# 91Mrwu/sif-xco2-cokriging

Hardware: AMD Instinct MI355X
Metric: cokriging grid-points/s at n_obs=20k bivariate (higher is better)
Workload: dtype f64; 1 GPU; configs[2]: n_obs=20000/process (N=40000) SIF+XCO2-like residuals on the 0.05-degree CONUS lattice, haversine, full 2n x 2n solve, 8833-point 0.5-degree grid, Matern set A; n_obs=20000, N=40000, m=8833, partition=block-column-cyclic x1

## Files before the change

sif-xco2-cokriging_amd/csrc/ck_api.hip:

```cpp
#include <hip/hip_runtime.h>
#include <math.h>
#include <stdio.h>
#include <string.h>

#include <algorithm>
#include <cmath>
#include <atomic>
#include <memory>
#include <string>
#include <utility>
#include <thread>
#include <vector>

#include "../../include/cokrige.h"
#include "ck_devbuf.h"
#include "ck_host.h"
#include "ck_internal.h"
#include "ck_tilemap.h"
#include "ck_model.h"
#include "ck_vecchia.h"

static int64_t roundup(int64_t x, int64_t a) { return (x + a - 1) / a * a; }
#define CK_N_TIMINGS 118
#define CK_TREND_TOL 1e-10
// ... 111 lines not shown
    int64_t p_cap = 0;
    DevBuf<char[24]> mv_buf;
    AuxState aux_state = AUX_NONE;
    double par_sigma[2] = {0.0, 0.0}, par_rho = 0.0;
    DevBuf<CkMatern> d_lik_blk;
    CkMatern lik_hb[15];
    DevBuf<double> baux;
    int64_t block_chunk = 0;
    int64_t sim_free_bytes = 0;
    int64_t draw_chunk = 0;
    struct Schur {
        int64_t M = 0;
        int tiles = 0;
        std::vector<DevBuf<double>> panels;
        std::vector<double*> sig;
        DevBuf<double*> d_ptr, d_coefptr;
        DevBuf<int> d_tile0, d_panel_of;
        DevBuf<double> pc, c, u;
        DevBuf<CkMatern> d_blk;
        DevBuf<CkTable> d_tabs;
        DevBuf<long long> d_info;
    } sch;
    std::vector<double> vg_ci, vg_cj, vg_vi, vg_vj;
    struct Vario {
        DevBuf<double> iu, iv, ju_own, jv_own;
        double *ju = nullptr, *jv = nullptr;
        DevBuf<unsigned long long> best;
        DevBuf<double> jb, ib64, jbsub;
        DevBuf<CkVarioExt> part;
        DevBuf<double> psum;
        DevBuf<unsigned long long> pcnt;
        DevBuf<double> out;
        DevBuf<CkVarioPair> list;
        DevBuf<unsigned> count;
    } vg;
    int64_t vg_ni = 0, vg_nj = 0;
    int vg_same = 0, vg_bgrid = 0;
    int64_t vg_stats[4] = {0, 0, 0, 0};
    double t_ms[CK_N_TIMINGS] = {};
    int time_gemm = 0;
    std::vector<EvPair> gemm_ev;
    size_t gemm_ev_used = 0;
    hipEvent_t ev0 = nullptr, ev1 = nullptr, ev2 = nullptr, ev3 = nullptr;
    hipStream_t side = nullptr;
    hipStream_t side_lo = nullptr;
    int fused_sweeps_opt = -1;
    int fused_prio = 0;
    int fused_group = 0;
    int group_first = -1, group_tail = 0, group_tail_panels = 0;
    int assemble_queue = -1;
    int tall_sweep = 1;
    int tall_split = 2;
    int tall_split_rows = 24 * CK_NB;
    int solve_la = -1;
    int tall_b2_stream = 1;
    std::vector<hipEvent_t> ev_b2;
    int tall_thin = 1;
    int fused_la = -1;
    std::vector<hipEvent_t> ev_col, ev_pan;
    int panel_group = 0;
    int64_t local_slab_mb = 0;
    int local_tile_min = 64;
    int64_t local_nmax[2] = {0, 0};
    int local_select_cap = 0;
    int local_group = 4;
    int local_left = 1;
    int panel_fused = 2 | 16;
    int64_t loo_g0 = -1;
    DevBuf<double> d_chunkb;
    DevBuf<double> local_slab;
    int lookahead = -1;
    DevBuf<unsigned> d_coop;
    DevBuf<unsigned long long> d_stamps;
    size_t n_stamps = 0;
    int64_t stamp_grid[4] = {0, 0, 0, 0};
    int stamp_sel = 0;
    unsigned coop_seq = 0;
    unsigned coop_spins = 2000000;
    int coop_inject_panel = -1;
    std::vector<double> trend_F[2];
    int trend_p[2] = {0, 0};
    bool trend_dirty = false;
    DevBuf<double> d_trendX;
    DevBuf<double> d_univ;
    std::vector<double> noise_var[2];
    double noise_scale[2] = {1.0, 1.0};
    bool noise_dirty = false, noise_on = false;
    DevBuf<double> d_noise;
    double lik_noise_grad[2] = {0.0, 0.0};
    bool lik_noise_valid = false;
    int aux_trend = 0;
    int loo_dense = 1;
    int64_t fisher_product_mb = 0;

    ~ck_handle() {
        for (auto& e : gemm_ev) {
            (void)hipEventDestroy(e.a);
            (void)hipEventDestroy(e.b);
        }
        for (hipEvent_t e : {ev0, ev1, ev2, ev3})
            if (e) (void)hipEventDestroy(e);
        for (const auto* v : {&ev_b2, &ev_col, &ev_pan})
            for (hipEvent_t e : *v) (void)hipEventDestroy(e);
        for (hipStream_t st : {side, side_lo, own_stream})
            if (st) (void)hipStreamDestroy(st);
    }
// ... 682 lines not shown
}
static void gemm_timed_end(ck_handle* h, hipStream_t st = nullptr) {
    if (!st) st = h->stream;
    if (!h->time_gemm) return;
    (void)hipEventRecord(h->gemm_ev[h->gemm_ev_used].b, st);
    h->gemm_ev_used++;
}

static void gemm_timed_collect(ck_handle* h, int slot, hipEvent_t ref = nullptr) {
    if (!h->time_gemm) return;
    double tot = 0;
    std::vector<std::pair<float, float>> iv;
    for (size_t e = 0; e < h->gemm_ev_used; ++e) {
        tot += elapsed_ms(h->gemm_ev[e].a, h->gemm_ev[e].b);
        if (ref) iv.push_back({(float)elapsed_ms(ref, h->gemm_ev[e].a), (float)elapsed_ms(ref, h->gemm_ev[e].b)});
    }
    h->t_ms[slot] = tot;
    h->t_ms[slot + 1] = (double)h->gemm_ev_used;
    if (ref) {
        std::sort(iv.begin(), iv.end());
        double un = 0, cs = 0, ce = -1;
        for (const auto& x : iv) {
            if (x.first > ce) {
                if (ce >= 0) un += ce - cs;
                cs = x.first;
                ce = x.second;
            } else if (x.second > ce) {
                ce = x.second;
            }
        }
        if (ce >= 0) un += ce - cs;
        h->t_ms[15] = un;
    }
    h->gemm_ev_used = 0;
}

static void sigma_update_on(ck_handle* h, hipStream_t st, int K0, int np, int J0, int Jstep, int nJ, bool timed) {
    unsigned long long* stamps = nullptr;
    if (h->d_stamps) {
        const size_t wgs = (size_t)((h->Npad - (int64_t)J0 * CK_NB) / 128) * (CK_NB / 128) * (size_t)nJ;
        if (wgs <= h->n_stamps && (h->stamp_sel == 1 || (nJ > 1 && K0 == h->stamp_sel - 2))) {
            stamps = h->d_stamps;
            h->stamp_grid[0] = (int64_t)ck_tilemap_make(h->nend, J0, Jstep, nJ).total;
            h->stamp_grid[1] = 1;
            h->stamp_grid[2] = J0;
            h->stamp_grid[3] = np;
        }
    }
    if (timed) gemm_timed_begin(h, st);
    ck_launch_syrk_group(st, h->d_sigptr, h->d_panelptr, K0, np, J0, Jstep, nJ, h->Npad, h->nend, stamps);
    if (timed) gemm_timed_end(h, st);
}

static void panel_factor_on(ck_handle* h, int K, hipStream_t st, bool with_aux = false, bool split = false) {
    double* P = h->sig[K];
    const int64_t R = h->Npad - (int64_t)K * CK_NB;
    double* tail = P + R * CK_NB;
    if (h->panel_fused & 16) {
        h->coop_seq += 1;
        int drop = -1;
        if (h->coop_inject_panel == K) {
            drop = 3;
            h->coop_inject_panel = -1;
        }
        double* X = with_aux ? h->aux + (int64_t)K * h->mpad * CK_NB : nullptr;
        if (split && with_aux && R > CK_NB) {
            ck_launch_panel_coop(st, P, CK_NB, tail, (int64_t)K * CK_NB, h->d_info, h->d_coop, h->coop_seq, h->d_coop + 16, nullptr, 0,
                                 h->coop_spins, drop);
            ck_launch_panel_rows_all(st, P + (int64_t)CK_NB * CK_NB, R - CK_NB, P, tail, X, h->mpad);
            return;
        }
        ck_launch_panel_coop(st, P, R, tail, (int64_t)K * CK_NB, h->d_info, h->d_coop, h->coop_seq, h->d_coop + 16, X, with_aux ? h->mpad : 0,
                             h->coop_spins, drop);
        return;
    }
    if (h->panel_fused & 4) {
        const int64_t RD = std::min<int64_t>(R, CK_NB);
        for (int q = 0; q < CK_NB / CK_IB; ++q) {
            double* diag = P + (int64_t)q * CK_IB * CK_NB + q * CK_IB;
            double* linv = tail + (int64_t)q * CK_IB * CK_IB;
            ck_launch_potrf64(st, diag, CK_NB, (int64_t)K * CK_NB + q * CK_IB, h->d_info, linv);
            const int64_t r1 = (int64_t)(q + 1) * CK_IB;
            if (RD > r1) ck_launch_trsm64(st, P + r1 * CK_NB + q * CK_IB, CK_NB, RD - r1, linv);
            const int64_t ncols = CK_NB - r1;
            if (ncols > 0 && RD > r1) {
                const int64_t ra = r1 / CK_BM * CK_BM;
                ck_launch_gemm_nt(st, P + ra * CK_NB + r1, CK_NB, P + ra * CK_NB + q * CK_IB, CK_NB,
                                  P + r1 * CK_NB + q * CK_IB, CK_NB, RD - ra, ncols, CK_IB, 1, ra - r1, 1, 0, 0, 0);
            }
        }
        if (R > CK_NB) ck_launch_panel_rows_all(st, P + (int64_t)CK_NB * CK_NB, R - CK_NB, P, tail);
        return;
    }
    if (h->panel_fused & 1) {
        for (int q = 0; q < CK_NB / CK_IB; ++q) {
            double* linv = tail + (int64_t)q * CK_IB * CK_IB;
            ck_launch_panel_diag(st, P, q, (int64_t)K * CK_NB, h->d_info, linv);
            const int64_t r1 = (int64_t)(q + 1) * CK_IB;
            ck_launch_panel_rows(st, P, r1, R - r1, P, q, linv);
        }
        return;
    }
    for (int q = 0; q < CK_NB / CK_IB; ++q) {
        double* diag = P + (int64_t)q * CK_IB * CK_NB + q * CK_IB;
        double* linv = tail + (int64_t)q * CK_IB * CK_IB;
        ck_launch_potrf64(st, diag, CK_NB, (int64_t)K * CK_NB + q * CK_IB, h->d_info, linv);
        const int64_t r1 = (int64_t)(q + 1) * CK_IB;
        ck_launch_trsm64(st, P + r1 * CK_NB + q * CK_IB, CK_NB, R - r1, linv);
        const int64_t ncols = CK_NB - r1;
        if (ncols > 0) {
            const int64_t ra = r1 / CK_BM * CK_BM;
            ck_launch_gemm_nt(st, P + ra * CK_NB + r1, CK_NB, P + ra * CK_NB + q * CK_IB, CK_NB,
                              P + r1 * CK_NB + q * CK_IB, CK_NB, R - ra, ncols, CK_IB, 1, ra - r1, 1, 0, 0, 0);
        }
    }
}

static void apply_sigma_on(ck_handle* h, int K, const double* P, int Jlo, int Jhi, hipStream_t st, bool timed) {
    int J0 = Jlo;
    while (J0 <= Jhi && (J0 % h->world) != h->rank) ++J0;
    if (J0 > Jhi) return;
    const int nJ = (Jhi - J0) / h->world + 1;
    (void)P;
    sigma_update_on(h, st, K, 1, J0, h->world, nJ, timed);
}

static int64_t aux_rows(const ck_handle* h, int K) {
    if (h->loo_g0 < 0) return h->mpad;
    const int64_t live = (int64_t)(K + 1) * CK_NB - h->loo_g0 + h->loo_dense;
    return std::min(h->mpad, roundup(std::max<int64_t>(live, 1), CK_AUX_ALIGN));
}

static int64_t aux_live(const ck_handle* h) { return h->loo_g0 < 0 && h->tall_thin ? h->m + 1 + h->aux_trend : 0; }

static void aux_group_on(ck_handle* h, hipStream_t st, int K0, int np, int J0, int nJ, bool timed) {
    if (nJ <= 0) return;
    if (timed) gemm_timed_begin(h, st);
    ck_launch_aux_group(st, h->aux, h->mpad, h->d_panelptr, K0, np, J0, nJ, aux_rows(h, K0 + np - 1), h->nend, aux_live(h));
    if (timed) gemm_timed_end(h, st);
}

static void aux_inner_on(ck_handle* h, int K, const double* P, hipStream_t st) {
    double* X = h->aux + (int64_t)K * h->mpad * CK_NB;
    const double* tail = P + (h->Npad - (int64_t)K * CK_NB) * CK_NB;
    const int64_t rows = aux_rows(h, K);
    if (h->panel_fused & 2) {
        ck_launch_panel_rows_all(st, X, rows, P, tail);
        return;
    }
    for (int q = 0; q < CK_NB / CK_IB; ++q) {
        ck_launch_trsm64(st, X + q * CK_IB, CK_NB, rows, tail + (int64_t)q * CK_IB * CK_IB);
        const int64_t r1 = (int64_t)(q + 1) * CK_IB;
        const int64_t ncols = CK_NB - r1;
        if (ncols > 0)
            ck_launch_gemm_nt(st, X + r1, CK_NB, X + q * CK_IB, CK_NB, P + r1 * CK_NB + q * CK_IB, CK_NB, rows,
                              ncols, CK_IB, 0, 0, 1, 0, 0, 0);
    }
}

static void aux_update_on(ck_handle* h, int K, const double* P, int Jlo, int Jhi, hipStream_t st, bool timed) {
    (void)P;
    aux_group_on(h, st, K, 1, Jlo, Jhi - Jlo + 1, timed && h->time_gemm == 1);
}

static int ensure_events(ck_handle* h) {
    while ((int)h->ev_col.size() < h->nK + 1) {
        hipEvent_t a, b;
        HIPCHK(hipEventCreateWithFlags(&a, hipEventDisableTiming));
        HIPCHK(hipEventCreateWithFlags(&b, hipEventDisableTiming));
        h->ev_col.push_back(a);
        h->ev_pan.push_back(b);
    }
    while ((int)h->ev_b2.size() < h->nK + 1) {
        hipEvent_t a;
        HIPCHK(hipEventCreateWithFlags(&a, hipEventDisableTiming));
        h->ev_b2.push_back(a);
    }
    return 0;
}

extern "C" int ck_panel_factor(ck_handle* h, int K) {
    CHKH(h);
    if (!h->assembled) return fail("ck_assemble_joint has not been called");
    if (K < 0 || K >= h->nK) return fail("bad panel index");
    if (!h->sig[K]) return fail("panel " + std::to_string(K) + " is not owned by this rank");
    panel_factor_on(h, K, h->stream);
    HIPCHK(hipGetLastError());
    return 0;
}

extern "C" int ck_panel_apply(ck_handle* h, int K, int what) {
    CHKH(h);
    if (K < 0 || K >= h->nK) return fail("bad panel index");
    const double* P = panel_src(h, K);
    if (what & CK_APPLY_SIGMA) apply_sigma_on(h, K, P, K + 1, h->nK - 1, h->stream, true);
    if ((what & CK_APPLY_AUX) && h->mpad > 0) {
        aux_inner_on(h, K, P, h->stream);
        aux_update_on(h, K, P, K + 1, h->nK - 1, h->stream, true);
    }
    HIPCHK(hipGetLastError());
// ... 3810 lines not shown
        if (value < -1 || value > 1) return fail("fused_sweeps must be -1 (automatic), 0 or 1");
        h->fused_sweeps_opt = (int)value;
        return 0;
    }
    if (!strcmp(name, "fused_prio")) {
        if (value < 0 || value > 2) return fail("fused_prio must be 0, 1 or 2");
        h->fused_prio = (int)value;
        return 0;
    }
    if (!strcmp(name, "coop_spins")) {
        if (value < 1000 || value > 2000000000LL) return fail("coop_spins must be in [1000, 2e9]");
        h->coop_spins = (unsigned)value;
        return 0;
    }
    if (!strcmp(name, "coop_inject_panel")) {
        if (value < -1) return fail("coop_inject_panel must be -1 (off) or a panel index");
        h->coop_inject_panel = (int)value;
        return 0;
    }
    if (!strcmp(name, "group_first") || !strcmp(name, "group_tail") || !strcmp(name, "group_tail_panels")) {
        if (value < (strcmp(name, "group_first") ? 0 : -1) || value > 1024) return fail("group_first (-1 = automatic) / group_tail / group_tail_panels must be in [0, 1024]");
        (!strcmp(name, "group_first") ? h->group_first : !strcmp(name, "group_tail") ? h->group_tail : h->group_tail_panels) = (int)value;
        return 0;
    }
    if (!strcmp(name, "assemble_queue")) {
        if (value < -1 || value > 4096) return fail("assemble_queue must be in [-1, 4096]");
        h->assemble_queue = (int)value;
        return 0;
    }
    if (!strcmp(name, "local_left")) {
        if (value < 0 || value > 1) return fail("local_left must be 0 or 1");
        h->local_left = (int)value;
        return 0;
    }
    if (!strcmp(name, "tall_split")) {
        if (value < 0 || value > 2) return fail("tall_split must be 0, 1 or 2");
        h->tall_split = (int)value;
        return 0;
    }
    if (!strcmp(name, "solve_la")) {
        if (value < -1 || value > 1) return fail("solve_la must be -1, 0 or 1");
        h->solve_la = (int)value;
        return 0;
    }
    if (!strcmp(name, "tall_b2_stream")) {
        h->tall_b2_stream = value != 0;
        return 0;
    }
    if (!strcmp(name, "tall_thin")) {
        if (value < 0 || value > 1) return fail("tall_thin must be 0 or 1");
        h->tall_thin = (int)value;
        return 0;
    }
    if (!strcmp(name, "tall_split_rows")) {
        if (value < 0) return fail("tall_split_rows must be >= 0");
        h->tall_split_rows = (int)std::min<int64_t>(value, 1 << 30);
        return 0;
    }
    if (!strcmp(name, "tall_sweep")) {
        if (value < 0 || value > 1) return fail("tall_sweep must be 0 or 1");
        h->tall_sweep = (int)value;
        return 0;
    }
    if (!strcmp(name, "fused_la")) {
        if (value < -1 || value > 1) return fail("fused_la must be -1 (automatic), 0 or 1");
        h->fused_la = (int)value;
        return 0;
    }
    if (!strcmp(name, "fused_group")) {
        if (value < 0 || value > 16) return fail("fused_group must be in [0, 16]");
        h->fused_group = (int)value;
        return 0;
    }
    if (!strcmp(name, "lookahead")) {
        if (value < -1 || value > 1) return fail("lookahead must be -1 (automatic), 0 or 1");
        h->lookahead = (int)value;
        return 0;
    }
    if (!strcmp(name, "local_slab_mb")) {
        if (value < 0) return fail("local_slab_mb must be >= 0");
        h->local_slab_mb = value;
        return 0;
    }
    if (!strcmp(name, "panel_fused")) {
        if (value < 0 || value > 31) return fail("panel_fused must be in [0, 31]");
        h->panel_fused = (int)value;
        return 0;
    }
    if (!strcmp(name, "local_group")) {
        if (value < 1 || value > CK_LT_NINV) return fail("local_group must be in [1, 8]");
        h->local_group = (int)value;
        return 0;
    }
    if (!strcmp(name, "local_select_cap")) {
        if (value < 1 || value > ck_local_select_capacity())
            return fail("local_select_cap must be in [1, " + std::to_string(ck_local_select_capacity()) + "]");
        h->local_select_cap = (int)value;
        return 0;
    }
    if (!strcmp(name, "local_tile_min")) {
        if (value < 0) return fail("local_tile_min must be >= 0");
        h->local_tile_min = (int)std::min<int64_t>(value, 1 << 30);
        return 0;
    }
    if (!strcmp(name, "panel_group")) {
        if (value < 0 || value > 16) return fail("panel_group must be in [0, 16] (0 = automatic)");
// ... 81 lines not shown
```

sif-xco2-cokriging_amd/csrc/ck_internal.h:

```cpp
#pragma once
#include <hip/hip_runtime.h>
#include <stdint.h>

#include "ck_host.h"
#include "ck_math.h"
#include "ck_vecchia_grad.h"
#include "ck_vecchia_info.h"
#include "ck_vecchia_trend.h"

#define CK_NB 512
#define CK_IB 64
#define CK_BM 256
#define CK_AUX_ALIGN 256
#define CK_PANEL_TAIL ((CK_NB / CK_IB) * CK_IB * CK_IB)

void ck_launch_prep_sites(hipStream_t s, const double* coords, int64_t n, int metric, double* c0, double* c1,
                          double* c2, double* u );
void ck_launch_table_nodes(hipStream_t s, const CkMatern* m, int metric, const double* q, int64_t n, double* out);
void ck_launch_table_check(hipStream_t s, const CkMatern* m, int metric, CkTable tab, const double* coef,
                           unsigned long long* max_err_bits);
struct CkLayout {
    long n0, n0p, nend, npad;
};
struct CkWorklist {
// ... 13 lines not shown
};
void ck_launch_assemble_sigma(hipStream_t s, bool fast, const CkMatern* blk, const CkTable* tabs,
                              const double* const* coefs, int metric, const double* c, const double* u, CkLayout L,
                              CkPanelMap pm, int total_tiles, CkWorklist wl, int queue_slots = 0 );
void ck_launch_assemble_aux(hipStream_t s, bool fast, const CkMatern* blk, const CkTable* tabs,
                            const double* const* coefs, int metric, int i_pred, double* pc, double* pu,
                            int64_t m, int64_t mpad, const double* c, const double* u, const double* z, CkLayout L,
                            int n_panels, double* aux, CkWorklist wl, const double* raw = nullptr, int queue_slots = 0);
void ck_launch_assemble_fix(hipStream_t s, bool aux_rows, const CkMatern* blk, int metric, int i_pred,
                            const double* pc, int64_t mpad, const double* c, CkLayout L, CkWorklist wl,
                            double* const* sigptr, double* aux);
void ck_launch_assemble_noise(hipStream_t s, double* const* sigptr, const double* nz, CkLayout L);
void ck_launch_cov_dense(hipStream_t s, const CkMatern* blk_ij, int metric, int add_nugget, int mode,
                         const double* a0, const double* a1, const double* a2, int64_t a, const double* b0,
                         const double* b1, const double* b2, int64_t b, double* out);
void ck_launch_model_variogram(hipStream_t s, const CkMatern* blk, double sill, int kind, const int* pi,
                               const int* pj, const double* lags, int64_t n, double* out);
void ck_launch_cov_lags(hipStream_t s, const CkMatern* blk_ij, int add_nugget, const double* lags, int64_t n,
                        double* out);

void ck_launch_block_fold(hipStream_t s, const double* aux, int64_t mpad, int n_panels, double* out, int64_t mpad_r,
                          const int* off, const int* rows, const double* w, int64_t r, int64_t zrow, int first);
#define CK_PRIOR_PIECE 512
void ck_launch_block_prior(hipStream_t s, const CkMatern* blk, int metric, const double* c0, const double* c1,
                           const double* c2, const double* w, const int* off, int64_t r, int full, const long long* poff,
                           int64_t n_pieces, double* part, double* diag, double* const* panels);

void ck_launch_gemm_nt(hipStream_t s, double* C, int64_t ldc, const double* A, int64_t lda, const double* B,
                       int64_t ldb, int64_t M, int64_t N, int64_t K, int lower, int64_t diag_off, int batch,
                       int64_t sC, int64_t sA, int64_t sB);
void ck_launch_cu_probe(hipStream_t s, unsigned* out, int n_wg, int spin);
void ck_launch_syrk_group(hipStream_t s, double* const* sigptr_dev, double* const* srcptr_dev, int K0, int np, int J0,
                          int Jstep, int nJ, int64_t Npad, int64_t nvalid ,
                          unsigned long long* stamps = nullptr );
void ck_launch_panel_coop(hipStream_t s, double* P, int64_t nrows, double* tail, int64_t g0, long long* info, unsigned* flags,
                          unsigned seq, unsigned* err, double* X = nullptr, int64_t xrows = 0, unsigned spins = 2000000u,
                          int drop = -1 );
void ck_launch_tall_group(hipStream_t s, double* const* sigptr_dev, double* aux, int64_t mpad, int K0, int np, int J0, int nJ,
                          int64_t nvalid, int64_t mrows = 0);
void ck_launch_panel_coop_prof(hipStream_t s, double* P, int64_t nrows, double* tail, int64_t g0, long long* info,
                               unsigned* flags, unsigned seq, unsigned* err, long long* prof);
void ck_launch_aux_group(hipStream_t s, double* aux, int64_t mpad, double* const* sigptr_dev, int K0, int np, int J0,
                         int nJ, int64_t mrows, int64_t nvalid, int64_t live_rows = 0);
void ck_launch_schur_syrk(hipStream_t s, double* const* schur_dev, const double* aux, int64_t mpad, int np, int nJ,
                          int64_t Mpad);
void ck_launch_ginv_syrk(hipStream_t s, double* const* G_dev, const double* aux, int64_t mpad, const double* avec, int nK,
                         int64_t nvalid, int q = 1, int64_t ald = 0, int dense = 1);
void ck_launch_draw_trmm(hipStream_t s, double* X, int64_t m, const double* E, int64_t ldp, int64_t nd, double* const* L_dev,
                         const double* pred, const double* ones, const int* cmap);
void ck_launch_potrf64(hipStream_t s, double* A, int64_t ld, int64_t global_index0, long long* info_dev,
                       double* Linv);
void ck_launch_potrf64_prof(hipStream_t s, double* A, int64_t ld, long long* info, double* Linv, long long* prof);
void ck_launch_panel_diag(hipStream_t s, double* P, int j, int64_t g0, long long* info, double* Linv);
void ck_launch_panel_rows_all(hipStream_t s, double* X, int64_t nrows, const double* P, const double* tail, double* X2 = nullptr,
                              int64_t nrows2 = 0);
void ck_launch_panel_rows(hipStream_t s, double* X, int64_t row_first, int64_t nrows, const double* P, int j,
                          const double* Linv);
void ck_launch_trsm64(hipStream_t s, double* A, int64_t ld, int64_t nrows, const double* Linv);
void ck_launch_reduce_pred(hipStream_t s, const double* aux, int64_t mpad, int n_panels, int64_t m, int64_t zrow,
                           double c0, double* pred, double* err);
void ck_launch_tri_matvec(hipStream_t s, double* const* sigptr_dev, int64_t npad, const double* v, double* out);
void ck_launch_loo_rows(hipStream_t s, double* aux, int64_t mpad, int64_t m, int64_t g0, const double* z,
                        int64_t npad, int64_t dense = 1);
#define CK_UNIV_QMAX 17
void ck_launch_reduce_univ(hipStream_t s, const double* aux, int64_t mpad, int n_panels, int64_t nrows, int64_t brow0, int q,
                           double* out);
void ck_launch_mfma_probe(hipStream_t s, int32_t* out);
int ck_launch_mfma_peak(hipStream_t s, int blocks, int waves_per_simd, int iters, double* sink);

void ck_launch_lik_logdet(hipStream_t s, double* const* sigptr_dev, int nK, CkLayout L, double* part);
#define CK_LIK_NPAR 11
int64_t ck_lik_grad_groups(CkLayout L);
void ck_launch_loglik_grad(hipStream_t s, double* const* G_dev, CkLayout L, int n_procs, int metric, const double* c,
                           const CkMatern* blk5, const double* dnu3, double sig1, double sig2, double rho, double* part);

void ck_launch_lik_noise_grad(hipStream_t s, double* const* G_dev, int nK, CkLayout L, const double* d, double* part);

#define CK_FISHER_NPAR 13
static_assert(CK_FISHER_NPAR == CK_LIK_NPAR + 2, "the model parameters and the two noise scales");
#define CK_FISHER_NOPS 13
#define CK_FISHER_NPAIR (CK_FISHER_NOPS * (CK_FISHER_NOPS + 1) / 2)
#define CK_FOP_R00 0
#define CK_FOP_R11 4
#define CK_FOP_R01 8
#define CK_FOP_DIAG0 11
#define CK_FISHER_YROWS 256
struct CkFisherUnit {
    double* D;
    long c0, wpad, nlo, nhi;
    int pK0, npan;
};
struct CkFisherAsm {
    double* D[CK_FOP_DIAG0][2];
    long c0[2], wpad[2];
    int pK0[2];
};
#define CK_FOPK_NONE 0
#define CK_FOPK_DENSE 1
#define CK_FOPK_DIAG0 2
struct CkFisherOp {
    const double* B;
    long ld, c0, w;
    int kind;
};
struct CkFisherOps {
    CkFisherOp op[CK_FISHER_NOPS];
    unsigned mask[CK_FISHER_NOPS];
};
// ... 195 lines not shown
```

sif-xco2-cokriging_amd/csrc/ck_la.hip:

```cpp
#include "ck_internal.h"
#include "ck_tilemap.h"

typedef double d4_t __attribute__((ext_vector_type(4)));
typedef double d2_t __attribute__((ext_vector_type(2)));

#define GEMM_BK 16

typedef __attribute__((address_space(1))) char ck_gchar;
typedef __attribute__((address_space(1))) double ck_gdouble;
typedef __attribute__((address_space(1))) d2_t ck_gd2;
__device__ __forceinline__ const ck_gchar* as_global(const char* p) { return (const ck_gchar*)(unsigned long long)p; }
__device__ __forceinline__ ck_gchar* as_global(char* p) { return (ck_gchar*)(unsigned long long)p; }

template <int WN>
__device__ __forceinline__ void gemm_tile(double* __restrict__ C, long ldc, const double* __restrict__ A, long lda,
                                          const double* __restrict__ B, long ldb, long r0, long c0, int K,
                                          char* lds) {
    constexpr int BN = WN * 32;
    constexpr int BCH = BN * 8 / 512;
    constexpr int PLANE_A = CK_BM * 16;
    constexpr int PLANE_B = BN * 16;
    constexpr int BOFF = 8 * PLANE_A;
    constexpr int STAGE = 8 * (PLANE_A + PLANE_B);

// ... 991 lines not shown
                                                  double* __restrict__ Linv) {
    __shared__ __attribute__((aligned(16))) double Lt[64][66];
    __shared__ __attribute__((aligned(16))) double Wi[64][66];
    potrf64_body(A, ld, g0, info, Linv, Lt, Wi);
}

void ck_launch_potrf64(hipStream_t s, double* A, int64_t ld, int64_t global_index0, long long* info_dev,
                       double* Linv) {
    k_potrf64<<<dim3(1), dim3(256), 0, s>>>(A, ld, global_index0, info_dev, Linv);
}

__device__ __forceinline__ void trsm64_body(double* __restrict__ A, long ld, long row0,
                                            const double* __restrict__ Linv) {
    constexpr int PITCH = 66;
    __shared__ __attribute__((aligned(16))) double As[64 * PITCH];
    __shared__ __attribute__((aligned(16))) double Li[64 * PITCH];
    const int tid = threadIdx.x, lane = tid & 63, w = tid >> 6;
    for (int idx = tid; idx < 64 * 64; idx += 256) {
        const int r = idx >> 6, c = idx & 63;
        As[r * PITCH + c] = A[(row0 + r) * ld + c];
        Li[r * PITCH + c] = Linv[idx];
    }
    __syncthreads();
    const int li = lane & 15, g = lane >> 4;
#pragma unroll
    for (int jt = 0; jt < 4; ++jt) {
        d4_t acc = {0.0, 0.0, 0.0, 0.0};
#pragma unroll
        for (int s = 0; s < 4 * (jt + 1); ++s) {
            const double av = As[(16 * w + li) * PITCH + 4 * s + g];
            const double bv = Li[(16 * jt + li) * PITCH + 4 * s + g];
            acc = __builtin_amdgcn_mfma_f64_16x16x4f64(av, bv, acc, 0, 0, 0);
        }
#pragma unroll
        for (int r = 0; r < 4; ++r) A[(row0 + 16 * w + g + 4 * r) * ld + 16 * jt + li] = acc[r];
    }
}

__global__ __launch_bounds__(256, 2) void k_trsm64m(double* __restrict__ A, long ld, long nrows,
                                                     const double* __restrict__ Linv) {
    trsm64_body(A, ld, (long)blockIdx.x * 64, Linv);
}

void ck_launch_trsm64(hipStream_t s, double* A, int64_t ld, int64_t nrows, const double* Linv) {
    if (nrows <= 0) return;
    k_trsm64m<<<dim3((unsigned)(nrows / 64)), dim3(256), 0, s>>>(A, ld, nrows, Linv);
}

template <bool COH>
__device__ __forceinline__ double ld_shared_result(const double* p) {
    return COH ? __hip_atomic_load(p, __ATOMIC_RELAXED, __HIP_MEMORY_SCOPE_AGENT) : *p;
}

template <bool SOLVE, bool COH = false, bool PUB = false>
__device__ __forceinline__ void lt_rows_body(double* __restrict__ C, const double* __restrict__ Ar, long ld,
                                             const double* __restrict__ Br, long ldb, int i,
                                             const double* __restrict__ Linv, double* As, double* Bs) {
    static_assert(!COH, "the coherent variant lives in k_panel_coop's own body");
    constexpr int PITCH = 66;
    typedef unsigned v4u_t __attribute__((ext_vector_type(4)));
    const int tid = threadIdx.x, lane = tid & 63, li = lane & 15, g = lane >> 4;
    const int w = __builtin_amdgcn_readfirstlane(tid >> 6);
    const int srow = tid >> 5, scp = tid & 31;
    const __amdgpu_buffer_rsrc_t rsA = __builtin_amdgcn_make_buffer_rsrc((void*)Ar, (short)0, 0x7fffffff, 0x00020000);
    const __amdgpu_buffer_rsrc_t rsB = __builtin_amdgcn_make_buffer_rsrc((void*)Br, (short)0, 0x7fffffff, 0x00020000);
    const __amdgpu_buffer_rsrc_t rsL = __builtin_amdgcn_make_buffer_rsrc((void*)Linv, (short)0, 0x7fffffff, 0x00020000);
    const int a_vo = (srow * (int)ld + 2 * scp) * 8, b_vo = (srow * (int)ldb + 2 * scp) * 8, l_vo = (srow * 64 + 2 * scp) * 8;
    const int a_rs = 8 * (int)ld * 8, b_rs = 8 * (int)ldb * 8;
    double* const As_w = As + srow * PITCH + 2 * scp;
    double* const Bs_w = Bs + srow * PITCH + 2 * scp;
    v4u_t ra[8], rb[8];
    if (i > 0) {
#pragma unroll
        for (int u = 0; u < 8; ++u) {
            ra[u] = __builtin_amdgcn_raw_buffer_load_b128(rsA, a_vo, u * a_rs, 0);
            rb[u] = __builtin_amdgcn_raw_buffer_load_b128(rsB, b_vo, u * b_rs, 0);
        }
    }
    d4_t cn[4];
#pragma unroll
    for (int jt = 0; jt < 4; ++jt)
#pragma unroll
        for (int r = 0; r < 4; ++r) cn[jt][r] = -C[(long)(16 * w + g + 4 * r) * ld + 16 * jt + li];
    for (int ks = 0; ks < i; ++ks) {
#pragma unroll
        for (int u = 0; u < 8; ++u) {
            *reinterpret_cast<v4u_t*>(As_w + 8 * u * PITCH) = ra[u];
            *reinterpret_cast<v4u_t*>(Bs_w + 8 * u * PITCH) = rb[u];
        }
        __syncthreads();
        if (ks + 1 < i) {
            const int so = 64 * (ks + 1) * 8;
#pragma unroll
            for (int u = 0; u < 8; ++u) {
                ra[u] = __builtin_amdgcn_raw_buffer_load_b128(rsA, a_vo, so + u * a_rs, 0);
                rb[u] = __builtin_amdgcn_raw_buffer_load_b128(rsB, b_vo, so + u * b_rs, 0);
            }
        } else if (SOLVE) {
#pragma unroll
            for (int u = 0; u < 8; ++u) rb[u] = __builtin_amdgcn_raw_buffer_load_b128(rsL, l_vo, u * (8 * 64 * 8), 0);
        }
#pragma unroll
        for (int s2 = 0; s2 < 16; ++s2) {
            const double av = As[(16 * w + li) * PITCH + 4 * s2 + g];
#pragma unroll
            for (int jt = 0; jt < 4; ++jt)
                cn[jt] = __builtin_amdgcn_mfma_f64_16x16x4f64(av, Bs[(16 * jt + li) * PITCH + 4 * s2 + g], cn[jt], 0, 0, 0);
        }
        __syncthreads();
    }
    if (!SOLVE) {
#pragma unroll
        for (int jt = 0; jt < 4; ++jt)
#pragma unroll
            for (int r = 0; r < 4; ++r) C[(long)(16 * w + g + 4 * r) * ld + 16 * jt + li] = -cn[jt][r];
        return;
    }
    if (i == 0) {
#pragma unroll
        for (int u = 0; u < 8; ++u) rb[u] = __builtin_amdgcn_raw_buffer_load_b128(rsL, l_vo, u * (8 * 64 * 8), 0);
    }
#pragma unroll
    for (int jt = 0; jt < 4; ++jt)
#pragma unroll
        for (int r = 0; r < 4; ++r) As[(16 * w + g + 4 * r) * PITCH + 16 * jt + li] = cn[jt][r];
#pragma unroll
    for (int u = 0; u < 8; ++u) *reinterpret_cast<v4u_t*>(Bs_w + 8 * u * PITCH) = rb[u];
    __syncthreads();
#pragma unroll
    for (int jt = 0; jt < 4; ++jt) {
        d4_t acc = {0.0, 0.0, 0.0, 0.0};
#pragma unroll
        for (int s2 = 0; s2 < 4 * (jt + 1); ++s2)
            acc = __builtin_amdgcn_mfma_f64_16x16x4f64(As[(16 * w + li) * PITCH + 4 * s2 + g],
                                                      Bs[(16 * jt + li) * PITCH + 4 * s2 + g], acc, 0, 0, 0);
#pragma unroll
        for (int r = 0; r < 4; ++r) st_shared_result<PUB>(C + (long)(16 * w + g + 4 * r) * ld + 16 * jt + li, -acc[r]);
    }
}

__device__ __forceinline__ void lt_diag_update(double* __restrict__ S, long ld, int g0, int i, double* M) {
    constexpr int PITCH = 66;
    const int tid = threadIdx.x, lane = tid & 63, w = tid >> 6, li = lane & 15, g = lane >> 4;
    const int jb = g0 + 64 * i;
    const double* Ar = S + (long)jb * ld + g0;
    double* C = S + (long)jb * ld + jb;
    const int sr = tid >> 6, sc = tid & 63;
    d4_t acc[4];
#pragma unroll
    for (int jt = 0; jt < 4; ++jt) acc[jt] = d4_t{0.0, 0.0, 0.0, 0.0};
    for (int ks = 0; ks < i; ++ks) {
        if (ks) __syncthreads();
#pragma unroll
        for (int u = 0; u < 16; ++u) M[(sr + 4 * u) * PITCH + sc] = Ar[(long)(sr + 4 * u) * ld + 64 * ks + sc];
        __syncthreads();
#pragma unroll
        for (int s2 = 0; s2 < 16; ++s2) {
            const double av = M[(16 * w + li) * PITCH + 4 * s2 + g];
#pragma unroll
            for (int jt = 0; jt < 4; ++jt)
                acc[jt] = __builtin_amdgcn_mfma_f64_16x16x4f64(av, M[(16 * jt + li) * PITCH + 4 * s2 + g], acc[jt], 0, 0, 0);
        }
    }
#pragma unroll
    for (int jt = 0; jt < 4; ++jt)
#pragma unroll
        for (int r = 0; r < 4; ++r) C[(long)(16 * w + g + 4 * r) * ld + 16 * jt + li] -= acc[jt][r];
}

__global__ __launch_bounds__(256, 3) void k_lt_potrf64(const CkLocalSys* __restrict__ sys, double* __restrict__ slab, int g0,
                                                     int i, long long* info) {
    __shared__ __attribute__((aligned(16))) double M[64][66];
    const CkLocalSys q = sys[blockIdx.x];
    double* S = slab + q.off;
    const int jb = g0 + 64 * i;
    if (i > 0) {
        lt_diag_update(S, q.ld, g0, i, &M[0][0]);
        __syncthreads();
    }
    potrf64_body<false, false>(S + (long)jb * q.ld + jb, q.ld, jb, info + blockIdx.x,
                               jb + 64 < q.kq ? S + (long)CK_LT_ROWS(q.kq) * q.ld + (long)i * 64 * 64 : nullptr, M, M);
}

__global__ __launch_bounds__(256, 2) void k_lt_rows(const CkLocalSys* __restrict__ sys, double* __restrict__ slab, int g0,
                                                     int i, int gb, const CkRunMap map) {
    __shared__ __attribute__((aligned(16))) double As[64 * 66];
    __shared__ __attribute__((aligned(16))) double Bs[64 * 66];
    int y, chunk;
    if (!ck_runmap_get(map, (int)blockIdx.x, y, chunk)) return;
    const CkLocalSys q = sys[y];
// ... 1 lines not shown
    const int lim = q.kq < g0 + 64 * gb ? q.kq : g0 + 64 * gb;
    const int nchunk = (lim - jb - 64) / 64;
    if (chunk >= nchunk) return;
    double* S = slab + q.off;
    const long row0 = jb + 64 + 64 * (long)chunk;
    lt_rows_body<true>(S + row0 * q.ld + jb, S + row0 * q.ld + g0, q.ld, S + (long)jb * q.ld + g0, q.ld, i,
                       S + (long)CK_LT_ROWS(q.kq) * q.ld + (long)i * 64 * 64, As, Bs);
}

__global__ __launch_bounds__(256, 2) void k_lt_rows_all(const CkLocalSys* __restrict__ sys, double* __restrict__ slab,
                                                         int g0, int gb, const CkRunMap map) {
    __shared__ __attribute__((aligned(16))) double As[64 * 66];
    __shared__ __attribute__((aligned(16))) double Bs[64 * 66];
    int y, chunk;
    if (!ck_runmap_get(map, (int)blockIdx.x, y, chunk)) return;
    const CkLocalSys q = sys[y];
    const int r_first = g0 + 64 * gb;
    const int nchunk = (q.kq - r_first) / 64;
    if (chunk >= nchunk) return;
    double* S = slab + q.off;
    const long row0 = r_first + 64 * (long)chunk;
    const double* linv = S + (long)CK_LT_ROWS(q.kq) * q.ld;
    for (int i = 0; i < gb; ++i) {
        if (i) {
            __threadfence_block();
            __syncthreads();
        }
        const int jb = g0 + 64 * i;
        lt_rows_body<true>(S + row0 * q.ld + jb, S + row0 * q.ld + g0, q.ld, S + (long)jb * q.ld + g0, q.ld, i,
                           linv + (long)i * 64 * 64, As, Bs);
    }
}

__global__ __launch_bounds__(256) void k_panel_diag(double* __restrict__ P, int j, long g0, long long* info,
                                                     double* __restrict__ Linv) {
    __shared__ __attribute__((aligned(16))) double M[64][66];
    const int jb = 64 * j;
    if (j > 0) {
        lt_diag_update(P, CK_NB, 0, j, &M[0][0]);
        __syncthreads();
    }
    potrf64_body(P + (long)jb * CK_NB + jb, CK_NB, g0 + jb, info, Linv, M, M);
}

__global__ __launch_bounds__(256, 2) void k_panel_rows(double* X, long row_first, const double* P,
                                                        int j, const double* __restrict__ Linv) {
    __shared__ __attribute__((aligned(16))) double As[64 * 66];
    __shared__ __attribute__((aligned(16))) double Bs[64 * 66];
    const int jb = 64 * j;
    const long row0 = row_first + 64 * (long)blockIdx.x;
    lt_rows_body<true>(X + row0 * CK_NB + jb, X + row0 * CK_NB, CK_NB, P + (long)jb * CK_NB, CK_NB, j, Linv, As, Bs);
}

__global__ __launch_bounds__(256, 2) void k_panel_rows_all(double* X, const double* P, const double* tail, double* X2, int n1) {
    __shared__ __attribute__((aligned(16))) double As[64 * 66];
    __shared__ __attribute__((aligned(16))) double Bs[64 * 66];
    const int b = (int)blockIdx.x;
    double* rows = b < n1 ? X + 64L * b * CK_NB : X2 + 64L * (b - n1) * CK_NB;
    for (int j = 0; j < CK_NB / 64; ++j) {
        if (j) {
            __threadfence_block();
            __syncthreads();
        }
        lt_rows_body<true>(rows + 64 * j, rows, CK_NB, P + (long)(64 * j) * CK_NB, CK_NB, j, tail + (long)j * 64 * 64, As, Bs);
    }
}

__device__ __forceinline__ bool coop_wait(const unsigned* flag, unsigned seq, unsigned* err, unsigned spins) {
    __shared__ int ok_s;
    __syncthreads();
    if (threadIdx.x == 0) {
        int ok = 0;
        for (unsigned spin = 0; spin < spins; ++spin) {
            if (__hip_atomic_load(flag, __ATOMIC_RELAXED, __HIP_MEMORY_SCOPE_AGENT) == seq) {
                ok = 1;
                break;
            }
            __builtin_amdgcn_s_sleep(2);
        }
        if (!ok) atomicOr(err, 1u);
        ok_s = ok;
    }
    __syncthreads();
    return ok_s != 0;
}

#define CK_SC1 16
#define CK_OWN 0
typedef unsigned ck_v4u_t __attribute__((ext_vector_type(4)));
typedef unsigned ck_v2u_t __attribute__((ext_vector_type(2)));
__device__ __forceinline__ __amdgpu_buffer_rsrc_t coop_rsrc(const double* p) {
    return __builtin_amdgcn_make_buffer_rsrc((void*)p, (short)0, 0x7fffffff, 0x00020000);
}
__device__ __forceinline__ double coop_as_double(ck_v2u_t v) {
    return __builtin_bit_cast(double, v);
}
__device__ __forceinline__ ck_v2u_t coop_as_v2u(double v) {
    return __builtin_bit_cast(ck_v2u_t, v);
}

__device__ __forceinline__ void coop_accumulate(d4_t (&cn)[4], const double* __restrict__ C, const double* __restrict__ Ar,
                                                const double* __restrict__ Br, int i, double* As, double* Bs) {
    constexpr int PITCH = 66;
    constexpr int LD = CK_NB;
    constexpr int RS = 8 * LD * 8;
    const int tid = threadIdx.x, lane = tid & 63, li = lane & 15, g = lane >> 4;
    const int w = __builtin_amdgcn_readfirstlane(tid >> 6);
    const int srow = tid >> 5, scp = tid & 31;
    const __amdgpu_buffer_rsrc_t rsA = coop_rsrc(Ar), rsB = coop_rsrc(Br), rsC = coop_rsrc(C);
    const int s_vo = (srow * LD + 2 * scp) * 8;
    const int c_vo = ((16 * w + g) * LD + li) * 8;
    double* const As_w = As + srow * PITCH + 2 * scp;
    double* const Bs_w = Bs + srow * PITCH + 2 * scp;
    ck_v4u_t ra[8], rb[8];
    if (i > 0) {
#pragma unroll
        for (int u = 0; u < 8; ++u) {
// ... 138 lines not shown
    double* D = rows + 64 * b;
    double (*M)[66] = reinterpret_cast<double (*)[66]>(As);
    __syncthreads();
#pragma unroll
    for (int jt = 0; jt < 4; ++jt)
#pragma unroll
        for (int r = 0; r < 4; ++r) M[16 * w + g + 4 * r][16 * jt + li] = -dacc[jt][r];
    __syncthreads();
    CK_COOP_MARK(5)
    potrf64_body<false, true, true, true>(D, CK_NB, g0 + 64 * b, info, tail + (long)b * 64 * 64, M, M);
    CK_COOP_MARK(6)
    asm volatile("s_waitcnt vmcnt(0)" ::: "memory");
    __syncthreads();
    if (threadIdx.x == 0 && drop != b) __hip_atomic_store(flags + b, seq, __ATOMIC_RELAXED, __HIP_MEMORY_SCOPE_AGENT);
    CK_COOP_MARK(7)
}

__global__ __launch_bounds__(256, 2) void k_panel_coop(double* P, double* tail, long g0, long long* info, unsigned* flags,
                                                        unsigned seq, unsigned* err, double* X, int nsig, unsigned spins, int drop) {
    __shared__ __attribute__((aligned(16))) double As[64 * 66];
    __shared__ __attribute__((aligned(16))) double Bs[64 * 66];
    const int b = (int)blockIdx.x;
    if (b < CK_NB / 64)
        panel_coop_body<false, true>(P, P + 64L * b * CK_NB, tail, g0, info, flags, seq, err, nullptr, As, Bs, spins, drop);
    else
        panel_coop_body<false, false>(P, b < nsig ? P + 64L * b * CK_NB : X + 64L * (b - nsig) * CK_NB, tail, g0, info, flags, seq,
                                      err, nullptr, As, Bs, spins, -1);
}

__global__ __launch_bounds__(256, 2) void k_panel_coop_prof(double* P, double* tail, long g0, long long* info, unsigned* flags,
                                                             unsigned seq, unsigned* err, long long* prof) {
    __shared__ __attribute__((aligned(16))) double As[64 * 66];
    __shared__ __attribute__((aligned(16))) double Bs[64 * 66];
    const int b = (int)blockIdx.x;
    if (b < CK_NB / 64)
        panel_coop_body<true, true>(P, P + 64L * b * CK_NB, tail, g0, info, flags, seq, err, prof, As, Bs, 2000000u, -1);
    else
        panel_coop_body<true, false>(P, P + 64L * b * CK_NB, tail, g0, info, flags, seq, err, prof, As, Bs, 2000000u, -1);
}

void ck_launch_panel_coop_prof(hipStream_t s, double* P, int64_t nrows, double* tail, int64_t g0, long long* info,
                               unsigned* flags, unsigned seq, unsigned* err, long long* prof) {
    k_panel_coop_prof<<<dim3((unsigned)(nrows / 64)), dim3(256), 0, s>>>(P, tail, (long)g0, info, flags, seq, err, prof);
}

void ck_launch_panel_coop(hipStream_t s, double* P, int64_t nrows, double* tail, int64_t g0, long long* info, unsigned* flags,
                          unsigned seq, unsigned* err, double* X, int64_t xrows, unsigned spins, int drop) {
    if (nrows <= 0) return;
    if (!X) xrows = 0;
    k_panel_coop<<<dim3((unsigned)((nrows + xrows) / 64)), dim3(256), 0, s>>>(P, tail, (long)g0, info, flags, seq, err, X,
                                                                              (int)(nrows / 64), spins, drop);
}

void ck_launch_panel_rows_all(hipStream_t s, double* X, int64_t nrows, const double* P, const double* tail, double* X2,
                              int64_t nrows2) {
    if (!X2) nrows2 = 0;
    if (nrows + nrows2 <= 0) return;
    k_panel_rows_all<<<dim3((unsigned)((nrows + nrows2) / 64)), dim3(256), 0, s>>>(X, P, tail, X2, (int)(nrows / 64));
}

void ck_launch_panel_diag(hipStream_t s, double* P, int j, int64_t g0, long long* info, double* Linv) {
    k_panel_diag<<<dim3(1), dim3(256), 0, s>>>(P, j, g0, info, Linv);
}

void ck_launch_panel_rows(hipStream_t s, double* X, int64_t row_first, int64_t nrows, const double* P, int j,
                          const double* Linv) {
    if (nrows <= 0) return;
    k_panel_rows<<<dim3((unsigned)(nrows / 64)), dim3(256), 0, s>>>(X, row_first, P, j, Linv);
}

__global__ __launch_bounds__(512, 4) void k_lt_update(const CkLocalSys* __restrict__ sys, double* __restrict__ slab,
                                                       int g0, int K, const CkRunMap map) {
    __shared__ __attribute__((aligned(16))) char lds[2 * 256 * 128];
    int y, t;
    if (!ck_runmap_get(map, (int)blockIdx.x, y, t)) return;
    const CkLocalSys q = sys[y];
    const int o = g0 + K;
    const int T = (q.kq - o + 127) / 128;
    if (t >= T * (T + 1) / 2) return;
    int tm = (int)((sqrtf(8.0f * (float)t + 1.0f) - 1.0f) * 0.5f);
    while (tm * (tm + 1) / 2 > t) --tm;
    while ((tm + 1) * (tm + 2) / 2 <= t) ++tm;
    const int tn = t - tm * (tm + 1) / 2;
    double* S = slab + q.off;
    const double* A = S + (long)o * q.ld + g0;
    gemm_tile_e<true>(S + (long)o * q.ld + o, q.ld, A, q.ld, A, q.ld, (long)tm * 128, (long)tn * 128, K, lds, q.kq - o, q.kq - o, true);
}

__global__ __launch_bounds__(512, 4) void k_lt_left(const CkLocalSys* __restrict__ sys, double* __restrict__ slab, int g0, int W,
                                                     const CkRunMap map) {
    __shared__ __attribute__((aligned(16))) char lds[2 * 256 * 128];
    int y, t;
    if (!ck_runmap_get(map, (int)blockIdx.x, y, t)) return;
    const CkLocalSys q = sys[y];
    const int rows = q.kq - g0;
    if (rows <= 0) return;
    const int w = rows < W ? rows : W;
    const int Tr = (rows + 127) / 128, Tc = (w + 127) / 128;
    const int ntile = Tr * Tc - (Tc == 2 ? 1 : 0);
    if (t >= ntile) return;
    int tm, tn;
    if (Tc == 1) {
        tm = t;
        tn = 0;
    } else if (t == 0) {
        tm = 0;
        tn = 0;
    } else {
        tm = (t + 1) >> 1;
        tn = (t + 1) & 1;
    }
// ... 285 lines not shown
```

Baseline: 18070 grid-points/s.

## Use 32-column K slabs in panel row-solve kernel to raise occupancy

Templates the panel row triangular-solve body on the K-slab width and makes 32 columns the default for k_panel_rows_all. The shared-memory tiles shrink to 64x34 and the launch bounds ask for four blocks per CU instead of two, which should give more latency hiding. The final triangular multiply by Linv is split into two halves with an extra barrier and accumulators kept across halves. The cost is twice as many slab iterations and barriers per block, and a more complex triangular epilogue. A rows_slab option still lets callers pick the old 64-column path.

```diff
diff --git a/sif-xco2-cokriging_amd/csrc/ck_api.hip b/sif-xco2-cokriging_amd/csrc/ck_api.hip
--- a/sif-xco2-cokriging_amd/csrc/ck_api.hip
+++ b/sif-xco2-cokriging_amd/csrc/ck_api.hip
@@ -187,6 +187,7 @@
     int tall_sweep = 1;
     int tall_split = 2;
     int tall_split_rows = 24 * CK_NB;
+    int rows_slab = 0;
     int solve_la = -1;
     int tall_b2_stream = 1;
     std::vector<hipEvent_t> ev_b2;
@@ -975,6 +976,8 @@
     if (timed) gemm_timed_end(h, st);
 }
 
+static int rows_slab(const ck_handle* h) { return h->rows_slab == 64 ? 64 : 32; }
+
 static void panel_factor_on(ck_handle* h, int K, hipStream_t st, bool with_aux = false, bool split = false) {
     double* P = h->sig[K];
     const int64_t R = h->Npad - (int64_t)K * CK_NB;
@@ -990,7 +993,7 @@
         if (split && with_aux && R > CK_NB) {
             ck_launch_panel_coop(st, P, CK_NB, tail, (int64_t)K * CK_NB, h->d_info, h->d_coop, h->coop_seq, h->d_coop + 16, nullptr, 0,
                                  h->coop_spins, drop);
-            ck_launch_panel_rows_all(st, P + (int64_t)CK_NB * CK_NB, R - CK_NB, P, tail, X, h->mpad);
+            ck_launch_panel_rows_all(st, P + (int64_t)CK_NB * CK_NB, R - CK_NB, P, tail, rows_slab(h), X, h->mpad);
             return;
         }
         ck_launch_panel_coop(st, P, R, tail, (int64_t)K * CK_NB, h->d_info, h->d_coop, h->coop_seq, h->d_coop + 16, X, with_aux ? h->mpad : 0,
@@ -1012,7 +1015,7 @@
                                   P + r1 * CK_NB + q * CK_IB, CK_NB, RD - ra, ncols, CK_IB, 1, ra - r1, 1, 0, 0, 0);
             }
         }
-        if (R > CK_NB) ck_launch_panel_rows_all(st, P + (int64_t)CK_NB * CK_NB, R - CK_NB, P, tail);
+        if (R > CK_NB) ck_launch_panel_rows_all(st, P + (int64_t)CK_NB * CK_NB, R - CK_NB, P, tail, rows_slab(h));
         return;
     }
     if (h->panel_fused & 1) {
@@ -1068,7 +1071,7 @@
     const double* tail = P + (h->Npad - (int64_t)K * CK_NB) * CK_NB;
     const int64_t rows = aux_rows(h, K);
     if (h->panel_fused & 2) {
-        ck_launch_panel_rows_all(st, X, rows, P, tail);
+        ck_launch_panel_rows_all(st, X, rows, P, tail, rows_slab(h));
         return;
     }
     for (int q = 0; q < CK_NB / CK_IB; ++q) {
@@ -4985,6 +4988,11 @@
         h->tall_thin = (int)value;
         return 0;
     }
+    if (!strcmp(name, "rows_slab")) {
+        if (value != 0 && value != 32 && value != 64) return fail("rows_slab must be 0, 32 or 64");
+        h->rows_slab = (int)value;
+        return 0;
+    }
     if (!strcmp(name, "tall_split_rows")) {
         if (value < 0) return fail("tall_split_rows must be >= 0");
         h->tall_split_rows = (int)std::min<int64_t>(value, 1 << 30);
diff --git a/sif-xco2-cokriging_amd/csrc/ck_internal.h b/sif-xco2-cokriging_amd/csrc/ck_internal.h
--- a/sif-xco2-cokriging_amd/csrc/ck_internal.h
+++ b/sif-xco2-cokriging_amd/csrc/ck_internal.h
@@ -89,8 +89,8 @@
                        double* Linv);
 void ck_launch_potrf64_prof(hipStream_t s, double* A, int64_t ld, long long* info, double* Linv, long long* prof);
 void ck_launch_panel_diag(hipStream_t s, double* P, int j, int64_t g0, long long* info, double* Linv);
-void ck_launch_panel_rows_all(hipStream_t s, double* X, int64_t nrows, const double* P, const double* tail, double* X2 = nullptr,
-                              int64_t nrows2 = 0);
+void ck_launch_panel_rows_all(hipStream_t s, double* X, int64_t nrows, const double* P, const double* tail, int slab,
+                              double* X2 = nullptr, int64_t nrows2 = 0);
 void ck_launch_panel_rows(hipStream_t s, double* X, int64_t row_first, int64_t nrows, const double* P, int j,
                           const double* Linv);
 void ck_launch_trsm64(hipStream_t s, double* A, int64_t ld, int64_t nrows, const double* Linv);
diff --git a/sif-xco2-cokriging_amd/csrc/ck_la.hip b/sif-xco2-cokriging_amd/csrc/ck_la.hip
--- a/sif-xco2-cokriging_amd/csrc/ck_la.hip
+++ b/sif-xco2-cokriging_amd/csrc/ck_la.hip
@@ -1067,27 +1067,32 @@
     return COH ? __hip_atomic_load(p, __ATOMIC_RELAXED, __HIP_MEMORY_SCOPE_AGENT) : *p;
 }
 
-template <bool SOLVE, bool COH = false, bool PUB = false>
+template <bool SOLVE, bool COH = false, bool PUB = false, int KS = 64>
 __device__ __forceinline__ void lt_rows_body(double* __restrict__ C, const double* __restrict__ Ar, long ld,
                                              const double* __restrict__ Br, long ldb, int i,
                                              const double* __restrict__ Linv, double* As, double* Bs) {
     static_assert(!COH, "the coherent variant lives in k_panel_coop's own body");
-    constexpr int PITCH = 66;
+    static_assert(KS == 64 || KS == 32, "K slabs of 64 or 32 columns");
+    constexpr int PITCH = KS + 2;
+    constexpr int NU = KS / 8;
+    constexpr int RG = 512 / KS;
+    constexpr int NH = 64 / KS;
+    constexpr int JH = KS / 16;
     typedef unsigned v4u_t __attribute__((ext_vector_type(4)));
     const int tid = threadIdx.x, lane = tid & 63, li = lane & 15, g = lane >> 4;
     const int w = __builtin_amdgcn_readfirstlane(tid >> 6);
-    const int srow = tid >> 5, scp = tid & 31;
+    const int srow = tid / (KS / 2), scp = tid % (KS / 2);
     const __amdgpu_buffer_rsrc_t rsA = __builtin_amdgcn_make_buffer_rsrc((void*)Ar, (short)0, 0x7fffffff, 0x00020000);
     const __amdgpu_buffer_rsrc_t rsB = __builtin_amdgcn_make_buffer_rsrc((void*)Br, (short)0, 0x7fffffff, 0x00020000);
     const __amdgpu_buffer_rsrc_t rsL = __builtin_amdgcn_make_buffer_rsrc((void*)Linv, (short)0, 0x7fffffff, 0x00020000);
     const int a_vo = (srow * (int)ld + 2 * scp) * 8, b_vo = (srow * (int)ldb + 2 * scp) * 8, l_vo = (srow * 64 + 2 * scp) * 8;
-    const int a_rs = 8 * (int)ld * 8, b_rs = 8 * (int)ldb * 8;
+    const int a_rs = RG * (int)ld * 8, b_rs = RG * (int)ldb * 8;
     double* const As_w = As + srow * PITCH + 2 * scp;
     double* const Bs_w = Bs + srow * PITCH + 2 * scp;
-    v4u_t ra[8], rb[8];
+    v4u_t ra[NU], rb[NU];
     if (i > 0) {
 #pragma unroll
-        for (int u = 0; u < 8; ++u) {
+        for (int u = 0; u < NU; ++u) {
             ra[u] = __builtin_amdgcn_raw_buffer_load_b128(rsA, a_vo, u * a_rs, 0);
             rb[u] = __builtin_amdgcn_raw_buffer_load_b128(rsB, b_vo, u * b_rs, 0);
         }
@@ -1097,26 +1102,27 @@
     for (int jt = 0; jt < 4; ++jt)
 #pragma unroll
         for (int r = 0; r < 4; ++r) cn[jt][r] = -C[(long)(16 * w + g + 4 * r) * ld + 16 * jt + li];
-    for (int ks = 0; ks < i; ++ks) {
-#pragma unroll
-        for (int u = 0; u < 8; ++u) {
-            *reinterpret_cast<v4u_t*>(As_w + 8 * u * PITCH) = ra[u];
-            *reinterpret_cast<v4u_t*>(Bs_w + 8 * u * PITCH) = rb[u];
+    const int nslab = NH * i;
+    for (int ks = 0; ks < nslab; ++ks) {
+#pragma unroll
+        for (int u = 0; u < NU; ++u) {
+            *reinterpret_cast<v4u_t*>(As_w + RG * u * PITCH) = ra[u];
+            *reinterpret_cast<v4u_t*>(Bs_w + RG * u * PITCH) = rb[u];
         }
         __syncthreads();
-        if (ks + 1 < i) {
-            const int so = 64 * (ks + 1) * 8;
-#pragma unroll
-            for (int u = 0; u < 8; ++u) {
+        if (ks + 1 < nslab) {
+            const int so = KS * (ks + 1) * 8;
+#pragma unroll
+            for (int u = 0; u < NU; ++u) {
                 ra[u] = __builtin_amdgcn_raw_buffer_load_b128(rsA, a_vo, so + u * a_rs, 0);
                 rb[u] = __builtin_amdgcn_raw_buffer_load_b128(rsB, b_vo, so + u * b_rs, 0);
             }
         } else if (SOLVE) {
 #pragma unroll
-            for (int u = 0; u < 8; ++u) rb[u] = __builtin_amdgcn_raw_buffer_load_b128(rsL, l_vo, u * (8 * 64 * 8), 0);
-        }
-#pragma unroll
-        for (int s2 = 0; s2 < 16; ++s2) {
+            for (int u = 0; u < NU; ++u) rb[u] = __builtin_amdgcn_raw_buffer_load_b128(rsL, l_vo, u * (RG * 64 * 8), 0);
+        }
+#pragma unroll
+        for (int s2 = 0; s2 < KS / 4; ++s2) {
             const double av = As[(16 * w + li) * PITCH + 4 * s2 + g];
 #pragma unroll
             for (int jt = 0; jt < 4; ++jt)
@@ -1133,24 +1139,58 @@
     }
     if (i == 0) {
 #pragma unroll
-        for (int u = 0; u < 8; ++u) rb[u] = __builtin_amdgcn_raw_buffer_load_b128(rsL, l_vo, u * (8 * 64 * 8), 0);
-    }
-#pragma unroll
-    for (int jt = 0; jt < 4; ++jt)
-#pragma unroll
-        for (int r = 0; r < 4; ++r) As[(16 * w + g + 4 * r) * PITCH + 16 * jt + li] = cn[jt][r];
-#pragma unroll
-    for (int u = 0; u < 8; ++u) *reinterpret_cast<v4u_t*>(Bs_w + 8 * u * PITCH) = rb[u];
-    __syncthreads();
-#pragma unroll
-    for (int jt = 0; jt < 4; ++jt) {
-        d4_t acc = {0.0, 0.0, 0.0, 0.0};
-#pragma unroll
-        for (int s2 = 0; s2 < 4 * (jt + 1); ++s2)
-            acc = __builtin_amdgcn_mfma_f64_16x16x4f64(As[(16 * w + li) * PITCH + 4 * s2 + g],
-                                                      Bs[(16 * jt + li) * PITCH + 4 * s2 + g], acc, 0, 0, 0);
-#pragma unroll
-        for (int r = 0; r < 4; ++r) st_shared_result<PUB>(C + (long)(16 * w + g + 4 * r) * ld + 16 * jt + li, -acc[r]);
+        for (int u = 0; u < NU; ++u) rb[u] = __builtin_amdgcn_raw_buffer_load_b128(rsL, l_vo, u * (RG * 64 * 8), 0);
+    }
+    if constexpr (KS == 64) {
+#pragma unroll
+        for (int jt = 0; jt < 4; ++jt)
+#pragma unroll
+            for (int r = 0; r < 4; ++r) As[(16 * w + g + 4 * r) * PITCH + 16 * jt + li] = cn[jt][r];
+#pragma unroll
+        for (int u = 0; u < 8; ++u) *reinterpret_cast<v4u_t*>(Bs_w + 8 * u * PITCH) = rb[u];
+        __syncthreads();
+#pragma unroll
+        for (int jt = 0; jt < 4; ++jt) {
+            d4_t acc = {0.0, 0.0, 0.0, 0.0};
+#pragma unroll
+            for (int s2 = 0; s2 < 4 * (jt + 1); ++s2)
+                acc = __builtin_amdgcn_mfma_f64_16x16x4f64(As[(16 * w + li) * PITCH + 4 * s2 + g],
+                                                          Bs[(16 * jt + li) * PITCH + 4 * s2 + g], acc, 0, 0, 0);
+#pragma unroll
+            for (int r = 0; r < 4; ++r) st_shared_result<PUB>(C + (long)(16 * w + g + 4 * r) * ld + 16 * jt + li, -acc[r]);
+        }
+    } else {
+        d4_t acc[4];
+#pragma unroll
+        for (int jt = 0; jt < 4; ++jt) acc[jt] = d4_t{0.0, 0.0, 0.0, 0.0};
+#pragma unroll
+        for (int h = 0; h < NH; ++h) {
+            if (h) __syncthreads();
+#pragma unroll
+            for (int jt = JH * h; jt < JH * (h + 1); ++jt)
+#pragma unroll
+                for (int r = 0; r < 4; ++r) As[(16 * w + g + 4 * r) * PITCH + 16 * (jt - JH * h) + li] = cn[jt][r];
+#pragma unroll
+            for (int u = 0; u < NU; ++u) *reinterpret_cast<v4u_t*>(Bs_w + RG * u * PITCH) = rb[u];
+            if (h + 1 < NH) {
+#pragma unroll
+                for (int u = 0; u < NU; ++u)
+                    rb[u] = __builtin_amdgcn_raw_buffer_load_b128(rsL, l_vo, KS * (h + 1) * 8 + u * (RG * 64 * 8), 0);
+            }
+            __syncthreads();
+#pragma unroll
+            for (int jt = JH * h; jt < 4; ++jt) {
+#pragma unroll
+                for (int s2 = 0; s2 < KS / 4; ++s2)
+                    if (KS / 4 * h + s2 < 4 * (jt + 1))
+                        acc[jt] = __builtin_amdgcn_mfma_f64_16x16x4f64(As[(16 * w + li) * PITCH + 4 * s2 + g],
+                                                                      Bs[(16 * jt + li) * PITCH + 4 * s2 + g], acc[jt], 0, 0, 0);
+                if (jt < JH * (h + 1)) {
+#pragma unroll
+                    for (int r = 0; r < 4; ++r) st_shared_result<PUB>(C + (long)(16 * w + g + 4 * r) * ld + 16 * jt + li, -acc[jt][r]);
+                }
+            }
+        }
     }
 }
 
@@ -1258,9 +1298,11 @@
     lt_rows_body<true>(X + row0 * CK_NB + jb, X + row0 * CK_NB, CK_NB, P + (long)jb * CK_NB, CK_NB, j, Linv, As, Bs);
 }
 
-__global__ __launch_bounds__(256, 2) void k_panel_rows_all(double* X, const double* P, const double* tail, double* X2, int n1) {
-    __shared__ __attribute__((aligned(16))) double As[64 * 66];
-    __shared__ __attribute__((aligned(16))) double Bs[64 * 66];
+template <int KS>
+__global__ __launch_bounds__(256, KS == 32 ? 4 : 2) void k_panel_rows_all(double* X, const double* P, const double* tail, double* X2,
+                                                                          int n1) {
+    __shared__ __attribute__((aligned(16))) double As[64 * (KS + 2)];
+    __shared__ __attribute__((aligned(16))) double Bs[64 * (KS + 2)];
     const int b = (int)blockIdx.x;
     double* rows = b < n1 ? X + 64L * b * CK_NB : X2 + 64L * (b - n1) * CK_NB;
     for (int j = 0; j < CK_NB / 64; ++j) {
@@ -1268,7 +1310,8 @@
             __threadfence_block();
             __syncthreads();
         }
-        lt_rows_body<true>(rows + 64 * j, rows, CK_NB, P + (long)(64 * j) * CK_NB, CK_NB, j, tail + (long)j * 64 * 64, As, Bs);
+        lt_rows_body<true, false, false, KS>(rows + 64 * j, rows, CK_NB, P + (long)(64 * j) * CK_NB, CK_NB, j, tail + (long)j * 64 * 64,
+                                             As, Bs);
     }
 }
 
@@ -1513,11 +1556,15 @@
                                                                               (int)(nrows / 64), spins, drop);
 }
 
-void ck_launch_panel_rows_all(hipStream_t s, double* X, int64_t nrows, const double* P, const double* tail, double* X2,
+void ck_launch_panel_rows_all(hipStream_t s, double* X, int64_t nrows, const double* P, const double* tail, int slab, double* X2,
                               int64_t nrows2) {
     if (!X2) nrows2 = 0;
     if (nrows + nrows2 <= 0) return;
-    k_panel_rows_all<<<dim3((unsigned)((nrows + nrows2) / 64)), dim3(256), 0, s>>>(X, P, tail, X2, (int)(nrows / 64));
+    const dim3 grid((unsigned)((nrows + nrows2) / 64));
+    if (slab == 64)
+        k_panel_rows_all<64><<<grid, dim3(256), 0, s>>>(X, P, tail, X2, (int)(nrows / 64));
+    else
+        k_panel_rows_all<32><<<grid, dim3(256), 0, s>>>(X, P, tail, X2, (int)(nrows / 64));
 }
 
 void ck_launch_panel_diag(hipStream_t s, double* P, int j, int64_t g0, long long* info, double* Linv) {
```

Measured after the change: 18170 grid-points/s (median of 6 runs). Within noise of the previous version (+0.5%).
